# MichaelAxtmann/InPlaceMSDradixsort

Measured on AMD Instinct MI355X. Metric: Gkeys/s + achieved HBM GB/s, 2^30 uniform u32 keys, 1/2/4/8 MI355X, higher is better.
Workload: dtype u32; 1 GPU; 2^30 uniform u32 keys per GPU, in-place MSD radix sort, 8-bit digits; config_id=c2, elements_per_gpu=1073741824, steps_verified=0, verified_by=not checked in a plain run (bench.py --full verifies every timed step), workspace_bytes=360054784

## Files before the change

### inplacemsdradixsort_amd/csrc/msd_count16.hpp

```cpp
#pragma once

namespace msd {

#ifndef MSD_C16_TH
#define MSD_C16_TH 512
#endif
constexpr int kC16Th = MSD_C16_TH;
constexpr int kC16Vec = 4096 / kC16Th;
constexpr int kC16Tail = 1024 / kC16Th;
constexpr uint32_t kC16Cap = kC16Th * (kC16Vec * 4 + kC16Tail);
constexpr uint32_t kC16MinBits = 9;
constexpr uint32_t kC16Words = 16384;
constexpr uint32_t kC16CwWords = kC16Words + (kC16Words >> 6) * 4;
static_assert(kC16CwWords == kC16Cap, "counters and output buffer share one LDS area");
constexpr size_t kC16Lds = (size_t)kC16Cap * 4 + kC16Th * 4 + 128 * 4 + 128;
__device__ __forceinline__ uint32_t c16_at(uint32_t w) { return w + ((w >> 6) << 2); }

__global__ __launch_bounds__(kC16Th, (kC16Th >= 1024 ? 8 : 4)) void count_place16_kernel(uint32_t *__restrict__ keys,
	const Segment *__restrict__ segs, uint32_t nsegs, Segment *__restrict__ rejected, Counters *__restrict__ ctr,
	uint64_t n_total)
{
	constexpr int TH = kC16Th, NV = kC16Vec, NT = kC16Tail, NK = NV * 4 + NT;
	constexpr int CH = TH >= 1024 ? 4 : 8;
	extern __shared__ __attribute__((aligned(16))) unsigned char smem[];
	uint32_t *cw = reinterpret_cast<uint32_t *>(smem);
	uint32_t *out = reinterpret_cast<uint32_t *>(smem);
	uint32_t *tbase = cw + kC16Cap;
	uint32_t *junkc = tbase + TH;
	uint32_t *junko = junkc + 64;
	uint32_t *wtot = junko + 64;
	uint32_t *nexti = wtot + 9, *hi_l = wtot + 10, *crowded = wtot + 11;
	const uint32_t tid = threadIdx.x, lane = tid & 63, w = tid >> 6;
	if (blockIdx.x >= nsegs) return;
	if (tid == 0) wtot[13] = 0;
	auto uniform = [](Segment g) -> Segment {
		Segment u;
		auto rfl = [](uint32_t x) -> uint64_t { return (uint64_t)(uint32_t)__builtin_amdgcn_readfirstlane(x); };
		u.start = rfl((uint32_t)g.start) | (rfl((uint32_t)(g.start >> 32)) << 32);
		u.count = rfl((uint32_t)g.count) | (rfl((uint32_t)(g.count >> 32)) << 32);
		u.bits = (uint32_t)rfl(g.bits);
		u.pad = 0;
		return u;
	};
	Segment sg = uniform(segs[blockIdx.x]);

	uint32_t rk[NK];
	auto prefetch = [&](const Segment &g) {
		const uint32_t off = (uint32_t)(g.start & 3u);
		const uint32_t *base = keys + (g.start - off);
		const uint64_t tot = g.count + off;
		const bool take = g.bits >= kC16MinBits && g.bits <= 16 && tot <= (uint64_t)kC16Cap && ((g.start - off + tot + 3) & ~3ull) <= n_total;
		const uint32_t totc = take ? (uint32_t)tot : 1u;
		const uint32_t lastv = (totc - 1u) >> 2;
#pragma unroll
		for (int v = 0; v < NV; ++v) {
			const u32x4 q = *reinterpret_cast<const u32x4 *>(base + min((uint32_t)(v * TH) + tid, lastv) * 4u);
			rk[v * 4 + 0] = q.x; rk[v * 4 + 1] = q.y; rk[v * 4 + 2] = q.z; rk[v * 4 + 3] = q.w;
		}
#pragma unroll
		for (int s = 0; s < NT; ++s) rk[NV * 4 + s] = base[min((uint32_t)(NV * TH * 4 + s * TH) + tid, totc - 1u)];
	};
	prefetch(sg);
	MSD_STAMP_DECL(2);
	MSD_STAMP_START();
	for (;;) {
		const uint32_t off = (uint32_t)(sg.start & 3u);
		const uint32_t tot = (uint32_t)min(sg.count + off, (uint64_t)0xFFFFFFFFu), n = tot - off;
		const bool fits = sg.bits >= kC16MinBits && sg.bits <= 16 && sg.count + off <= (uint64_t)kC16Cap && ((sg.start + sg.count + 3) & ~3ull) <= n_total;
		const uint32_t vsh = 16u - (fits ? sg.bits : 16u);
		uint32_t *segb = keys + (sg.start - off);
		MSD_STAMP(9);
		MSD_STAMP_TICK(11);
		uint32_t zero = 0, tq = tid;
		asm volatile("" : "+v"(zero), "+v"(tq));
#pragma unroll
		for (uint32_t j = 0; j < (kC16Cap / 4 + TH - 1) / TH; ++j) {
			const uint32_t q = j * TH + tq;
			if (q < kC16Cap / 4) reinterpret_cast<u32x4 *>(cw)[q] = u32x4{ zero, zero, zero, zero };
		}
		if (tid == 0) {
			if (wtot[13] == 0) {
				const uint32_t take = nsegs > 64u * gridDim.x ? 2u : 1u;
				wtot[12] = atomicAdd(&ctr->count_ticket3, take) + gridDim.x;
				wtot[13] = take;
			}
			*nexti = wtot[12];
			wtot[12] += 1;
			wtot[13] -= 1;
			*crowded = 0;
			const uint32_t k0 = off == 0 ? rk[0] : off == 1 ? rk[1] : off == 2 ? rk[2] : rk[3];
			*hi_l = k0 & ~((1u << sg.bits) - 1u);
		}
		MSD_STAMP(0);
		__syncthreads();
		MSD_STAMP(1);
		if (fits) {
#pragma unroll
			for (int u0 = 0; u0 < NK; u0 += CH) {
				uint32_t old[CH];
#pragma unroll
				for (int i = 0; i < CH; ++i) {
					const int u = u0 + i;
					if (u < NK) {
						const uint32_t el = u < NV * 4 ? (uint32_t)((u / 4) * TH * 4) + tid * 4 + (u % 4) : (uint32_t)(NV * TH * 4 + (u - NV * 4) * TH) + tid;
						const uint32_t val = (rk[u] << vsh) & 0xFFFFu;
						const bool in = el >= off && el < tot;
						const uint32_t a = in ? c16_at(val >> 2) : (uint32_t)(junkc - cw) + lane;
						old[i] = atomicAdd(cw + a, 1u << ((val & 3u) * 8u));
						rk[u] = val | (in ? 0u : 0x80000000u);
					}
				}
#pragma unroll
				for (int i = 0; i < CH; ++i) {
					const int u = u0 + i;
					if (u < NK) rk[u] |= ((old[i] >> ((rk[u] & 3u) * 8u)) & 0xFFu) << 16;
				}
				__builtin_amdgcn_sched_barrier(0);
			}
		}
		MSD_STAMP(2);
		__syncthreads();
		MSD_STAMP(3);
		const uint32_t nxt = (uint32_t)__builtin_amdgcn_readfirstlane(*nexti), hi = (uint32_t)__builtin_amdgcn_readfirstlane(*hi_l);
		const Segment nraw = segs[nxt < nsegs ? nxt : blockIdx.x];
		constexpr int WPT = (int)(kC16Words / TH);
		u32x4 *cq = reinterpret_cast<u32x4 *>(cw + c16_at(tid * (uint32_t)WPT));
		uint32_t cr[WPT];
		uint32_t totk = 0;
		if (fits) {
#pragma unroll
			for (int j = 0; j < WPT / 4; ++j) {
				const u32x4 q = cq[j];
				cr[4 * j + 0] = q.x; cr[4 * j + 1] = q.y; cr[4 * j + 2] = q.z; cr[4 * j + 3] = q.w;
			}
#pragma unroll
			for (int j = 0; j < WPT; ++j) totk = __builtin_amdgcn_sad_u8(cr[j], 0u, totk);
		}
		if (totk > 255u) *crowded = 1;
		const uint32_t inc = wave_incl_scan(totk);
		if ((tq & 63u) == 63u) wtot[tq >> 6] = inc;
		MSD_STAMP(4);
		__syncthreads();
		uint32_t pos = inc - totk, all = 0;
#pragma unroll
		for (uint32_t ww = 0; ww < TH / 64; ++ww) {
			const uint32_t t = wtot[ww];
			if (ww < w) pos += t;
			all += t;
		}
		const bool ok = fits && all == n && *crowded == 0;
		MSD_STAMP(5);
		if (ok) {
			uint32_t run = 0;
#pragma unroll
			for (int j = 0; j < WPT / 4; ++j) {
#pragma unroll
				for (int e = 0; e < 4; ++e) {
					const uint32_t x = cr[4 * j + e], y = x * 0x01010101u;
					cr[4 * j + e] = (y - x) + run * 0x01010101u;
					run += y >> 24;
				}
				cq[j] = u32x4{ cr[4 * j + 0], cr[4 * j + 1], cr[4 * j + 2], cr[4 * j + 3] };
			}
			tbase[tid] = pos + off;
			MSD_STAMP(6);
			__syncthreads();
#pragma unroll
			for (int u0 = 0; u0 < NK; u0 += CH) {
				uint32_t tb[CH], cv[CH];
#pragma unroll
				for (int i = 0; i < CH; ++i) {
					if (u0 + i < NK) {
						const uint32_t wi = (rk[u0 + i] & 0xFFFFu) >> 2;
						tb[i] = tbase[wi / (uint32_t)WPT];
						cv[i] = cw[c16_at(wi)];
					}
				}
#pragma unroll
				for (int i = 0; i < CH; ++i) {
					if (u0 + i < NK) {
						const uint32_t r = rk[u0 + i];
						const uint32_t pl = tb[i] + ((cv[i] >> ((r & 3u) * 8u)) & 0xFFu) + ((r >> 16) & 0xFFu);
						rk[u0 + i] = (r & 0x8000FFFFu) | (pl << 16);
					}
				}
				__builtin_amdgcn_sched_barrier(0);
			}
			MSD_STAMP(7);
			__syncthreads();
#pragma unroll
			for (int u = 0; u < NK; ++u) {
				uint32_t *o = (rk[u] >> 31) ? junko + lane : out + ((rk[u] >> 16) & 0x7FFFu);
				*o = hi | ((rk[u] & 0xFFFFu) >> vsh);
			}
			__syncthreads();
			MSD_STAMP(8);
		} else if (tid == 0)
			rejected[atomicAdd(&ctr->nslow16, 1u)] = sg;
		Segment nsg = sg;
		if (nxt < nsegs) {
			nsg = uniform(nraw);
			prefetch(nsg);
		}
		if (ok) {
			const uint32_t v_first = off ? 1u : 0u, v_end = tot >> 2;
#pragma unroll
			for (int v0 = 0; v0 < NV; v0 += 4) {
				u32x4 t4[4];
#pragma unroll
				for (int i = 0; i < 4; ++i) t4[i] = reinterpret_cast<const u32x4 *>(out)[(uint32_t)((v0 + i) * TH) + tid];
#pragma unroll
				for (int i = 0; i < 4; ++i) {
					const uint32_t q = (uint32_t)((v0 + i) * TH) + tid;
					if (q >= v_first && q < v_end) reinterpret_cast<u32x4 *>(segb)[q] = t4[i];
				}
				__builtin_amdgcn_sched_barrier(0);
			}
			{
				const uint32_t q = (uint32_t)(NV * TH) + tq;
				if (q < v_end) reinterpret_cast<u32x4 *>(segb)[q] = reinterpret_cast<const u32x4 *>(out)[q];
			}
			if (tq < 4) {
				if (off && tq >= off && tq < tot) segb[tq] = out[tq];
				const uint32_t el = (v_end << 2) + tq;
				if (el < tot && el >= off && (el >= 4u || !off)) segb[el] = out[el];
			}
		}
		MSD_STAMP(10);
		if (nxt >= nsegs) break;
		sg = nsg;
		__syncthreads();
	}
	MSD_STAMP_FLUSH(TH / 64);
}

}
```

Before: 146.6 Gkeys/s.

## Double-buffer key registers, fuse LDS clear into writeback, prefetch ticket early

Splits the per-thread key registers into two ping-pong buffers so the next segment is prefetched into the other buffer during the scan and placement phases instead of after them. The LDS counter area is now zeroed while the sorted output is written back, rather than in a separate pass at the start of each segment, which removes one barrier per segment. The work-stealing ticket is drawn at kernel start and refilled asynchronously mid-segment, taking the global atomic off the critical path. Edge elements are now written per element inside the main writeback loop. The second register buffer doubles key register use, which may lower occupancy or cause spills.

```diff
diff --git a/inplacemsdradixsort_amd/csrc/msd_count16.hpp b/inplacemsdradixsort_amd/csrc/msd_count16.hpp
--- a/inplacemsdradixsort_amd/csrc/msd_count16.hpp
+++ b/inplacemsdradixsort_amd/csrc/msd_count16.hpp
@@ -6,6 +6,12 @@
 #define MSD_C16_TH 512
 #endif
 constexpr int kC16Th = MSD_C16_TH;
+#ifndef MSD_C16_EARLY_TICKET
+#define MSD_C16_EARLY_TICKET 1
+#endif
+#ifndef MSD_C16_SV
+#define MSD_C16_SV 8
+#endif
 constexpr int kC16Vec = 4096 / kC16Th;
 constexpr int kC16Tail = 1024 / kC16Th;
 constexpr uint32_t kC16Cap = kC16Th * (kC16Vec * 4 + kC16Tail);
@@ -32,7 +38,15 @@
 	uint32_t *nexti = wtot + 9, *hi_l = wtot + 10, *crowded = wtot + 11;
 	const uint32_t tid = threadIdx.x, lane = tid & 63, w = tid >> 6;
 	if (blockIdx.x >= nsegs) return;
-	if (tid == 0) wtot[13] = 0;
+	constexpr bool kEarlyTicket = MSD_C16_EARLY_TICKET;
+	const uint32_t ntake = nsegs > 64u * gridDim.x ? 2u : 1u;
+	if (tid == 0) {
+		wtot[13] = 0;
+		if (kEarlyTicket) {
+			wtot[12] = atomicAdd(&ctr->count_ticket3, ntake) + gridDim.x;
+			wtot[13] = ntake;
+		}
+	}
 	auto uniform = [](Segment g) -> Segment {
 		Segment u;
 		auto rfl = [](uint32_t x) -> uint64_t { return (uint64_t)(uint32_t)__builtin_amdgcn_readfirstlane(x); };
@@ -44,26 +58,39 @@
 	};
 	Segment sg = uniform(segs[blockIdx.x]);
 
-	uint32_t rk[NK];
-	auto prefetch = [&](const Segment &g) {
+	uint32_t rka[NK], rkb[NK];
+	auto prefetch = [&](uint32_t (&rk)[NK], const Segment &g, bool live) __attribute__((always_inline)) {
+		uint32_t tp = tid;
+		asm volatile("" : "+v"(tp));
 		const uint32_t off = (uint32_t)(g.start & 3u);
 		const uint32_t *base = keys + (g.start - off);
 		const uint64_t tot = g.count + off;
-		const bool take = g.bits >= kC16MinBits && g.bits <= 16 && tot <= (uint64_t)kC16Cap && ((g.start - off + tot + 3) & ~3ull) <= n_total;
+		const bool take = live && g.bits >= kC16MinBits && g.bits <= 16 && tot <= (uint64_t)kC16Cap && ((g.start - off + tot + 3) & ~3ull) <= n_total;
 		const uint32_t totc = take ? (uint32_t)tot : 1u;
 		const uint32_t lastv = (totc - 1u) >> 2;
 #pragma unroll
 		for (int v = 0; v < NV; ++v) {
-			const u32x4 q = *reinterpret_cast<const u32x4 *>(base + min((uint32_t)(v * TH) + tid, lastv) * 4u);
+			const u32x4 q = *reinterpret_cast<const u32x4 *>(base + min((uint32_t)(v * TH) + tp, lastv) * 4u);
 			rk[v * 4 + 0] = q.x; rk[v * 4 + 1] = q.y; rk[v * 4 + 2] = q.z; rk[v * 4 + 3] = q.w;
 		}
 #pragma unroll
-		for (int s = 0; s < NT; ++s) rk[NV * 4 + s] = base[min((uint32_t)(NV * TH * 4 + s * TH) + tid, totc - 1u)];
-	};
-	prefetch(sg);
+		for (int s = 0; s < NT; ++s) rk[NV * 4 + s] = base[min((uint32_t)(NV * TH * 4 + s * TH) + tp, totc - 1u)];
+	};
+	auto clear_all = [&]() __attribute__((always_inline)) {
+		uint32_t zero = 0, tc = tid;
+		asm volatile("" : "+v"(zero), "+v"(tc));
+#pragma unroll
+		for (uint32_t j = 0; j < (kC16Cap / 4 + TH - 1) / TH; ++j) {
+			const uint32_t q = j * TH + tc;
+			if (q < kC16Cap / 4) reinterpret_cast<u32x4 *>(cw)[q] = u32x4{ zero, zero, zero, zero };
+		}
+	};
+	prefetch(rka, sg, true);
+	clear_all();
+	__syncthreads();
 	MSD_STAMP_DECL(2);
 	MSD_STAMP_START();
-	for (;;) {
+	auto segment = [&](uint32_t (&rk)[NK], uint32_t (&rn)[NK]) __attribute__((always_inline)) -> bool {
 		const uint32_t off = (uint32_t)(sg.start & 3u);
 		const uint32_t tot = (uint32_t)min(sg.count + off, (uint64_t)0xFFFFFFFFu), n = tot - off;
 		const bool fits = sg.bits >= kC16MinBits && sg.bits <= 16 && sg.count + off <= (uint64_t)kC16Cap && ((sg.start + sg.count + 3) & ~3ull) <= n_total;
@@ -73,16 +100,10 @@
 		MSD_STAMP_TICK(11);
 		uint32_t zero = 0, tq = tid;
 		asm volatile("" : "+v"(zero), "+v"(tq));
-#pragma unroll
-		for (uint32_t j = 0; j < (kC16Cap / 4 + TH - 1) / TH; ++j) {
-			const uint32_t q = j * TH + tq;
-			if (q < kC16Cap / 4) reinterpret_cast<u32x4 *>(cw)[q] = u32x4{ zero, zero, zero, zero };
-		}
 		if (tid == 0) {
-			if (wtot[13] == 0) {
-				const uint32_t take = nsegs > 64u * gridDim.x ? 2u : 1u;
-				wtot[12] = atomicAdd(&ctr->count_ticket3, take) + gridDim.x;
-				wtot[13] = take;
+			if (!kEarlyTicket && wtot[13] == 0) {
+				wtot[12] = atomicAdd(&ctr->count_ticket3, ntake) + gridDim.x;
+				wtot[13] = ntake;
 			}
 			*nexti = wtot[12];
 			wtot[12] += 1;
@@ -92,7 +113,6 @@
 			*hi_l = k0 & ~((1u << sg.bits) - 1u);
 		}
 		MSD_STAMP(0);
-		__syncthreads();
 		MSD_STAMP(1);
 		if (fits) {
 #pragma unroll
@@ -122,7 +142,11 @@
 		__syncthreads();
 		MSD_STAMP(3);
 		const uint32_t nxt = (uint32_t)__builtin_amdgcn_readfirstlane(*nexti), hi = (uint32_t)__builtin_amdgcn_readfirstlane(*hi_l);
-		const Segment nraw = segs[nxt < nsegs ? nxt : blockIdx.x];
+		const bool more = nxt < nsegs;
+		const Segment nraw = segs[more ? nxt : blockIdx.x];
+		const bool refill = kEarlyTicket && tid == 0 && wtot[13] == 0;
+		uint32_t drawn = 0;
+		if (refill) drawn = atomicAdd(&ctr->count_ticket3, ntake);
 		constexpr int WPT = (int)(kC16Words / TH);
 		u32x4 *cq = reinterpret_cast<u32x4 *>(cw + c16_at(tid * (uint32_t)WPT));
 		uint32_t cr[WPT];
@@ -163,6 +187,17 @@
 				cq[j] = u32x4{ cr[4 * j + 0], cr[4 * j + 1], cr[4 * j + 2], cr[4 * j + 3] };
 			}
 			tbase[tid] = pos + off;
+		} else if (tid == 0)
+			rejected[atomicAdd(&ctr->nslow16, 1u)] = sg;
+		__builtin_amdgcn_sched_barrier(0);
+		const Segment nsg = uniform(nraw);
+		prefetch(rn, nsg, more);
+		__builtin_amdgcn_sched_barrier(0);
+		if (refill) {
+			wtot[12] = drawn + gridDim.x;
+			wtot[13] = ntake;
+		}
+		if (ok) {
 			MSD_STAMP(6);
 			__syncthreads();
 #pragma unroll
@@ -195,41 +230,49 @@
 			}
 			__syncthreads();
 			MSD_STAMP(8);
-		} else if (tid == 0)
-			rejected[atomicAdd(&ctr->nslow16, 1u)] = sg;
-		Segment nsg = sg;
-		if (nxt < nsegs) {
-			nsg = uniform(nraw);
-			prefetch(nsg);
-		}
-		if (ok) {
 			const uint32_t v_first = off ? 1u : 0u, v_end = tot >> 2;
-#pragma unroll
-			for (int v0 = 0; v0 < NV; v0 += 4) {
-				u32x4 t4[4];
-#pragma unroll
-				for (int i = 0; i < 4; ++i) t4[i] = reinterpret_cast<const u32x4 *>(out)[(uint32_t)((v0 + i) * TH) + tid];
-#pragma unroll
-				for (int i = 0; i < 4; ++i) {
-					const uint32_t q = (uint32_t)((v0 + i) * TH) + tid;
-					if (q >= v_first && q < v_end) reinterpret_cast<u32x4 *>(segb)[q] = t4[i];
-				}
+			auto put = [&](uint32_t q, const u32x4 &t) __attribute__((always_inline)) {
+				if (q >= v_first && q < v_end)
+					reinterpret_cast<u32x4 *>(segb)[q] = t;
+				else if (q == v_end || q < v_first) {
+					const uint32_t e0 = q << 2;
+					if (e0 + 0 >= off && e0 + 0 < tot) segb[e0 + 0] = t.x;
+					if (e0 + 1 >= off && e0 + 1 < tot) segb[e0 + 1] = t.y;
+					if (e0 + 2 >= off && e0 + 2 < tot) segb[e0 + 2] = t.z;
+					if (e0 + 3 >= off && e0 + 3 < tot) segb[e0 + 3] = t.w;
+				}
+			};
+			constexpr int SV = MSD_C16_SV < NV ? MSD_C16_SV : NV;
+#pragma unroll
+			for (int v0 = 0; v0 < NV; v0 += SV) {
+				u32x4 t4[SV];
+#pragma unroll
+				for (int i = 0; i < SV; ++i) t4[i] = reinterpret_cast<const u32x4 *>(out)[(uint32_t)((v0 + i) * TH) + tq];
+#pragma unroll
+				for (int i = 0; i < SV; ++i) reinterpret_cast<u32x4 *>(out)[(uint32_t)((v0 + i) * TH) + tq] = u32x4{ zero, zero, zero, zero };
+#pragma unroll
+				for (int i = 0; i < SV; ++i) put((uint32_t)((v0 + i) * TH) + tq, t4[i]);
 				__builtin_amdgcn_sched_barrier(0);
 			}
 			{
 				const uint32_t q = (uint32_t)(NV * TH) + tq;
-				if (q < v_end) reinterpret_cast<u32x4 *>(segb)[q] = reinterpret_cast<const u32x4 *>(out)[q];
-			}
-			if (tq < 4) {
-				if (off && tq >= off && tq < tot) segb[tq] = out[tq];
-				const uint32_t el = (v_end << 2) + tq;
-				if (el < tot && el >= off && (el >= 4u || !off)) segb[el] = out[el];
-			}
-		}
+				if (q < kC16Cap / 4) {
+					const u32x4 t = reinterpret_cast<const u32x4 *>(out)[q];
+					reinterpret_cast<u32x4 *>(out)[q] = u32x4{ zero, zero, zero, zero };
+					put(q, t);
+				}
+			}
+		} else if (fits)
+			clear_all();
 		MSD_STAMP(10);
-		if (nxt >= nsegs) break;
+		if (!more) return false;
 		sg = nsg;
 		__syncthreads();
+		return true;
+	};
+	for (;;) {
+		if (!segment(rka, rkb)) break;
+		if (!segment(rkb, rka)) break;
 	}
 	MSD_STAMP_FLUSH(TH / 64);
 }
```

Measured after the change: 151.1 Gkeys/s (median of 6 runs). +3.0%, better.
